# JamesYang007/adelie

Measured on AMD Instinct MI355X. Metric: lambda-paths/sec (100-lambda grpnet); HBM GB/s vs peak, higher is better.
Workload: dtype f64

## Files before the change

### adelie_amd/csrc/common.hpp

```cpp
#pragma once
#include <cstdlib>
#include <algorithm>
#include <hip/hip_runtime.h>

#include <chrono>
#include <cstdint>
#include <cstring>
#include <mutex>
#include <stdexcept>
#include <string>
#include <vector>

#include "../../include/adelie_hip.h"
#include "kernels.hpp"
#include "dev_array_host.hpp"

namespace ahip {

struct Hooks {
    long long cd_block_min_nv = -1;
    int panel_bsz = 0;
    int sparse_panel = -1;
    int std_panel = -1;
    int lookahead = -1, speculate = -1;
    int factor_sweep = -1;
    int relu_sweep = -1;
    int filter_sweep = -1;
    int filter_depth = -1;
    double filter_depth_margin = -1;
    double irls_reuse = -1;
    bool time_panel = false;
    bool cons_host = false;
    int trace = 0;
    static Hooks from_env() {
        Hooks h;
        if (const char* e = std::getenv("ADELIE_HIP_CD_BLOCK_MIN_NV")) h.cd_block_min_nv = std::atoll(e);
        if (const char* e = std::getenv("ADELIE_HIP_PANEL_BSZ")) {
            const int v = std::atoi(e);
            h.panel_bsz = (v == 32 || v == 64 || v == 128) ? v : 0;
        }
        if (const char* e = std::getenv("ADELIE_HIP_LOOKAHEAD")) h.lookahead = std::atoi(e) != 0;
        if (const char* e = std::getenv("ADELIE_HIP_SPECULATE")) h.speculate = std::atoi(e) != 0;
        if (const char* e = std::getenv("ADELIE_HIP_IRLS_REUSE")) h.irls_reuse = std::max(0.0, std::atof(e));
        h.time_panel = std::getenv("ADELIE_HIP_TIME_PANEL") != nullptr;
        if (const char* e = std::getenv("ADELIE_HIP_CONS_HOST")) h.cons_host = std::atoi(e) != 0;
        if (const char* e = std::getenv("ADELIE_HIP_SPARSE_PANEL")) h.sparse_panel = std::atoi(e) != 0;
        if (const char* e = std::getenv("ADELIE_HIP_STD_PANEL")) h.std_panel = std::atoi(e) != 0;
        if (const char* e = std::getenv("ADELIE_HIP_TRACE")) h.trace = std::max(1, std::atoi(e));
        h.factor_sweep = factor_sweep_env();
        h.relu_sweep = relu_sweep_env();
        h.filter_sweep = filter_sweep_env();
        if (const char* e = std::getenv("ADELIE_HIP_FILTER_DEPTH")) h.filter_depth = std::atoi(e) != 0;
        if (const char* e = std::getenv("ADELIE_HIP_FILTER_DEPTH_MARGIN")) h.filter_depth_margin = std::max(0.0, std::atof(e));
        return h;
    }
    static int filter_sweep_env() {
        const char* e = std::getenv("ADELIE_HIP_FILTER_SWEEP");
        return e ? int(std::atoi(e) != 0) : -1;
    }
    static int shadow_kind_env() { return shadow_kind_parse(std::getenv("ADELIE_HIP_SHADOW_KIND")); }
    static int64_t shadow_min_bytes_env() {
        const char* e = std::getenv("ADELIE_HIP_SHADOW_MIN_BYTES");
        return e ? int64_t(std::atoll(e)) : kShadowMinBytesDefault;
    }
    static int factor_sweep_env() {
        const char* e = std::getenv("ADELIE_HIP_FACTOR_SWEEP");
        return e ? int(std::atoi(e) != 0) : -1;
    }
    static int relu_sweep_env() {
        const char* e = std::getenv("ADELIE_HIP_RELU_SWEEP");
        return e ? int(std::atoi(e) != 0) : -1;
    }
};
struct SweepHooks {
    int factor = -1, relu = -1;
    static SweepHooks from_env() { return SweepHooks{Hooks::factor_sweep_env(), Hooks::relu_sweep_env()}; }
};
constexpr bool kFactorSweepDefault = false;
inline bool factor_sweep_on(int hook) { return hook < 0 ? kFactorSweepDefault : hook != 0; }
constexpr bool kReluSweepDefault = true;
inline bool relu_sweep_on(int hook) { return hook < 0 ? kReluSweepDefault : hook != 0; }
constexpr bool kReluSparseSweepDefault = true;
inline bool relu_sparse_sweep_on(int hook) { return hook < 0 ? kReluSparseSweepDefault : hook != 0; }
constexpr bool kFilterSweepDefault = true;
inline bool filter_sweep_on(int hook) { return hook < 0 ? kFilterSweepDefault : hook != 0; }
constexpr bool kFilterDepthDefault = true;
inline bool filter_depth_on(int hook) { return hook < 0 ? kFilterDepthDefault : hook != 0; }


inline core_error make_core_error(const std::string& m) { return core_error("adelie_core: " + m); }
inline core_error make_solver_error(const std::string& m) { return core_error("adelie_core solver: " + m); }

#define AHIP_CHECK(expr)                                                                                   \
    do {                                                                                                   \
        hipError_t _e = (expr);                                                                            \
        if (_e != hipSuccess)                                                                              \
            throw ::ahip::core_error(std::string("adelie_hip: HIP error '") + hipGetErrorString(_e) +     \
                                     "' at " #expr);                                                       \
    } while (0)

struct DevAllocStats {
    static double& seconds() { static double s = 0; return s; }
    static long& calls() { static long c = 0; return c; }
};

struct HostPool {
    struct Entry { size_t bytes; unsigned flags; void* p; };
    static std::mutex& mu() { static std::mutex* m = new std::mutex; return *m; }
    static std::vector<Entry>& parked() { static auto* v = new std::vector<Entry>; return *v; }
    static void* take(size_t bytes, unsigned flags) {
// ... 462 lines not shown
```

### adelie_amd/csrc/filter_host.hpp

```cpp
#pragma once
#include <algorithm>
#include <cmath>
#include <cstdint>
#include <vector>

namespace ahip {

constexpr int kFilterRuleStrong = 0, kFilterRulePivot = 1;

inline int64_t pivot_need(int64_t old_size, int64_t n_new_active, int64_t G, double subset_ratio, int64_t subset_min,
                          double slack_ratio) {
    const int64_t subset_size =
        std::min<int64_t>(std::max<int64_t>(int64_t(double(old_size) * (1 + subset_ratio)), subset_min), G);
    return subset_size + int64_t(std::ceil(slack_ratio * double(n_new_active))) + old_size + 2;
}

struct FilterRule {
    int screen_rule = kFilterRulePivot;
    double alpha = 1, lm = 0, lm_next = 0;
    bool thr_valid = false;
    double screen_thr = 0;
    int64_t thr_count = 0;
    int64_t G = 0, screen_size = 0, n_new_active = 0;
    double subset_ratio = 0.1, slack_ratio = 1.25;
// ... 18 lines not shown
    return (tstar > 0 && std::isfinite(tstar)) ? tstar : 0;
}

template <class I, class T>
inline std::vector<int32_t> filter_unpenalized_cols(const std::vector<I>& groups, const std::vector<I>& group_sizes,
                                                    const std::vector<T>& penalty) {
    std::vector<int32_t> c;
    for (size_t g = 0; g < groups.size(); ++g)
        if (!(penalty[g] > 0))
            for (I t = 0; t < group_sizes[g]; ++t) c.push_back(int32_t(groups[g] + t));
    return c;
}

constexpr int32_t kFilterOverflow = 1, kFilterStale = 2;
struct FilterFollowUp {
    bool refill;
    bool retire;
};
inline FilterFollowUp filter_follow_up(int32_t flags) {
    return FilterFollowUp{(flags & (kFilterOverflow | kFilterStale)) != 0, (flags & kFilterStale) != 0};
}
inline int64_t filter_list_cap(int64_t p) { return std::max<int64_t>(1024, p / 4); }

}
```

### adelie_amd/csrc/kernels.hpp

```cpp
#pragma once
#include <hip/hip_runtime.h>
#include <cstdint>
#include "gram_shape.hpp"
#include "multi_shape.hpp"
#include "relu_shape.hpp"
#include "relu_sparse_shape.hpp"
#include "shadow_kind_host.hpp"
#include "pieces_host.hpp"

namespace ahip {

template <class T>
struct DenseView {
    const T* X;
    int64_t n, p, ld;
};
struct SnpView {
    const uint8_t* bits;
    int64_t n, p, ldb;
};

template <class T>
struct PiecesView {
    const void* base[kMaxPieces];
// ... 74 lines not shown
void launch_shadow_build_q15(const DenseView<double>& X, int16_t* Xq, int64_t lds, double* scale, double* err, double* nrm,
                             int32_t* bad, hipStream_t s);
int filter_norm_parts(int64_t n);
struct FilteredSweep {
    const double *w, *r;
    double* v;
    double* grad;
    const double *sub_scale, *sub_vec;
    const int32_t* screen_cols;
    int64_t n_screen_cols;
    const int32_t* pen0_cols;
    int64_t n_pen0_cols;
    const int64_t *groups, *group_sizes;
    int64_t G;
    const int32_t* slot;
    const double* penalty;
    double tstar;
    double* sq_part;
    int32_t* list;
    int64_t cap;
    int32_t* meta_i;
    double* meta_d;
    double* work;
};
int64_t filtered_sweep_work_elems(int64_t n, int64_t p, int64_t n_before, int64_t cap);
void enqueue_filtered_sweep(const DenseView<double>& X, const ShadowView& S, const FilteredSweep& a, hipStream_t s);
int64_t sweep_work_elems_csc(int nb, int64_t ncols);
template <class T>
void launch_sweep_csc(const CscView<T>& X, const T* v, T* out, int64_t c0, int64_t ncols, const int32_t* cols,
                      const T* sub_scale, const T* sub_vec, bool square, T* work, hipStream_t s);
constexpr int kVecSumScratch = 8 + 256;
template <class T> void launch_vec_sum(const T* v, int64_t n, T* out, hipStream_t s);
template <class T>
void launch_std_sweep_epilogue(const T* center, const T* inv_scale, const T* raw, const T* raw_plain, const T* vsum, bool square,
                               T* out, int64_t c0, int64_t ncols, const int32_t* cols, const T* sub_scale, const T* sub_vec,
                               hipStream_t s);
template <class T>
void launch_std_gram_fix(const T* center, const T* inv_scale, T* C, int64_t ldc, int32_t M, int32_t pos0, int32_t N,
                         const int32_t* vcol, const T* m, const T* wsum, const T* xm, bool centered, hipStream_t s);
template <class T>
void launch_std_scale_coef(const T* center, const T* inv_scale, const int32_t* cols, const T* coef, const int32_t* count_dev,
                           int32_t count, T* coef2, T* kappa, hipStream_t s);
template <class T> void launch_vec_shift(T* out, int64_t n, const T* kappa, T sign, const int32_t* count_dev, hipStream_t s);
template <class T>
void launch_std_fix_gblk(T* gblk, const int32_t* cols, int nb, const T* center, const T* inv_scale, const T* rsum_dev,
                         const T* xm_view_or_null, hipStream_t s);
// ... 574 lines not shown
```

### adelie_amd/csrc/kernels_filter.hip

```cpp
#include "sweep_common.hpp"
#include <algorithm>
#include <cfloat>

namespace ahip {

namespace {

__global__ __launch_bounds__(kThreads) void shadow_build_kernel(const double* __restrict__ X, int64_t ld, int64_t n,
                                                                float* __restrict__ Xs, int64_t lds, double* __restrict__ err,
                                                                double* __restrict__ nrm, int32_t* __restrict__ bad) {
    const int64_t j = blockIdx.x;
    const int tid = threadIdx.x;
    const double* col = X + j * ld;
    float* dst = Xs + j * lds;
    double e2 = 0, n2 = 0;
    bool any_bad = false;
    for (int64_t i = tid; i < lds; i += kThreads) {
        float f = 0.f;
        if (i < n) {
            const double x = col[i];
            const bool ok = fabs(x) <= double(FLT_MAX);
            any_bad = any_bad || !ok;
            f = ok ? float(x) : 0.f;
            const double d = x - double(f);
// ... 55 lines not shown
            const double t = fmin(fmax(rint(__dmul_rn(x, inv)), -32767.0), 32767.0);
            q = int(t);
            const double d = (x - __dmul_rn(sc, t)) / sc;
            e2 = fma(d, d, e2);
            q2 = fma(t, t, q2);
        }
        dst[i] = int16_t(q);
    }
    e2 = wave_sum(e2);
    q2 = wave_sum(q2);
    if (lane == 0) { red[0][wv] = e2; red[1][wv] = q2; }
    __syncthreads();
    if (tid == 0) {
        double a = 0, b = 0;
        for (int w = 0; w < kThreads / 64; ++w) { a += red[0][w]; b += red[1][w]; }
        scale[j] = sc;
        err[j] = (sc > 0 ? sc * sqrt(a) : sqrt(double(n)) * m) * (1.0 + 1e-9);
        nrm[j] = sc * sqrt(b) * (1.0 + 1e-9);
    }
    if (any_bad) atomicOr(bad, 1);
}

__global__ __launch_bounds__(kThreads) void vmul_sq_kernel(const double* __restrict__ a, const double* __restrict__ b,
                                                           double* __restrict__ out, int64_t n, double* __restrict__ part) {
    double acc = 0;
    for (int64_t i = int64_t(blockIdx.x) * blockDim.x + threadIdx.x; i < n; i += int64_t(gridDim.x) * blockDim.x) {
        const double x = a[i] * b[i];
        out[i] = x;
        acc = fma(x, x, acc);
    }
    __shared__ double red[kThreads / 64];
    const int lane = threadIdx.x & 63, wv = threadIdx.x >> 6;
    acc = wave_sum(acc);
    if (lane == 0) red[wv] = acc;
    __syncthreads();
    if (threadIdx.x == 0) {
        double s = 0;
        for (int w = 0; w < kThreads / 64; ++w) s += red[w];
        part[blockIdx.x] = s;
    }
}

__device__ __forceinline__ void shadow_guard(double exact, double approx, int64_t j, const double* __restrict__ err,
                                             const double* __restrict__ nrm, double fp_term, const double* __restrict__ vnorm,
                                             int32_t* __restrict__ flags) {
    const double bound = (err[j] + fp_term * nrm[j]) * vnorm[0];
    if (!(fabs(exact - approx) <= bound)) atomicOr(flags, 2);
}

template <int VEC>
__device__ __forceinline__ double list_column_sum(const DenseAcc<double>& X, const double* __restrict__ v, int64_t j, int64_t r0,
                                                  int64_t r1, double* red) {
    const int tid = threadIdx.x;
    const double* cp = X.colptr(j);
    double acc = 0;
    const int64_t body_end = r0 + ((r1 - r0) / VEC) * VEC;
#pragma unroll 8
    for (int64_t i = r0 + int64_t(tid) * VEC; i < body_end; i += int64_t(kThreads) * VEC) {
        const Pack<double, VEC> vv = load_vec<double, VEC>(v + i);
        const Pack<double, VEC> xx = X.template load<VEC>(cp, i, j);
#pragma unroll
        for (int e = 0; e < VEC; ++e) acc = fma(xx.v[e], vv.v[e], acc);
    }
    for (int64_t i = body_end + tid; i < r1; i += kThreads) acc = fma(X.template load<1>(cp, i, j).v[0], v[i], acc);
    const int lane = tid & 63, wv = tid >> 6;
    const double ws = wave_sum(acc);
    if (lane == 0) red[wv] = ws;
    __syncthreads();
    double s = 0;
    if (tid == 0) {
#pragma unroll
        for (int w = 0; w < kThreads / 64; ++w) s += red[w];
    }
    return s;
}

struct ShadowF32 {
    using elem = float;
    using vec = f4_t;
    static constexpr int CB = kShadowCB, VEC = kShadowVec, kUnroll = 2;
    static constexpr bool kScaled = false, kPipelined = false;
    static constexpr int kMinWaves = 1;
    static __device__ __forceinline__ double row(vec x, int e) { return double(x[e]); }
};
typedef int i4_t __attribute__((ext_vector_type(4)));
struct ShadowQ15 {
    using elem = int16_t;
    using vec = i4_t;
    static constexpr int CB = kShadowCB16, VEC = kShadowVec16;
    static constexpr bool kScaled = true, kPipelined = true;
    static constexpr int kMinWaves = 5;
    static_assert(VEC == 8, "one 16-byte load holds 8 rows");
    static __device__ __forceinline__ double row(vec x, int e) {
        return e % 2 ? double(x[e / 2] >> 16) : double(int(int16_t(x[e / 2])));
    }
};

// ... 162 lines not shown
            out[j] = s;
        } else {
            part[int64_t(split) * max_cols + c] = s;
        }
    }
}
__global__ void sweep_list_reduce_kernel(const double* __restrict__ part, double* __restrict__ out,
                                         const int32_t* __restrict__ cols, int64_t max_cols,
                                         const int32_t* __restrict__ count_dev, int nsplit, const double* __restrict__ sub_scale,
                                         const double* __restrict__ sub_vec, const double* __restrict__ err,
                                         const double* __restrict__ nrm, double fp_term, const double* __restrict__ vnorm,
                                         int32_t* __restrict__ flags) {
    const int64_t c = int64_t(blockIdx.x) * blockDim.x + threadIdx.x;
    const int64_t count = count_dev ? min(int64_t(count_dev[0]), max_cols) : max_cols;
    if (c >= count) return;
    const int64_t j = cols[c];
    double s = 0;
    for (int r = 0; r < nsplit; ++r) s += part[int64_t(r) * max_cols + c];
    s = centred(s, j, sub_scale, sub_vec);
    if (err) shadow_guard(s, out[j], j, err, nrm, fp_term, vnorm, flags);
    out[j] = s;
}

constexpr int kClassifyThreads = 1024, kClassifyRun = 6;
__global__ __launch_bounds__(kClassifyThreads) void filter_classify_kernel(
    double* __restrict__ grad, const int64_t* __restrict__ groups, const int64_t* __restrict__ group_sizes, int64_t G,
    const int32_t* __restrict__ slot, const double* __restrict__ penalty, double tstar, const double* __restrict__ err,
    const double* __restrict__ nrm, double fp_term, const double* __restrict__ sq_part, int n_part,
    const double* __restrict__ sub_scale, const double* __restrict__ sub_vec, const double* __restrict__ stage,
    const int32_t* __restrict__ xa, int64_t na, const int32_t* __restrict__ xb, int64_t nb, int x_nsplit,
    int32_t* __restrict__ list, int64_t cap, int32_t* __restrict__ meta_i, double* __restrict__ meta_d) {
    constexpr int NW = kClassifyThreads / 64, R = kClassifyRun;
    __shared__ double sred[NW];
    __shared__ int32_t wtot[NW];
    __shared__ double s_vnorm;
    __shared__ int32_t s_first[kClassifyThreads * R], s_want[kClassifyThreads * R];
    const int tid = threadIdx.x, lane = tid & 63, wv = tid >> 6;
    {
        double a = 0;
        for (int i = tid; i < n_part; i += kClassifyThreads) a += sq_part[i];
        a = wave_sum(a);
        if (lane == 0) sred[wv] = a;
        __syncthreads();
        if (tid == 0) {
            double s = 0;
            for (int w = 0; w < NW; ++w) s += sred[w];
            s_vnorm = sqrt(s) * (1.0 + 1e-6);
            meta_d[0] = s_vnorm;
            meta_d[1] = sub_scale ? sub_scale[0] : 0.0;
            meta_i[1] = 0;
            meta_i[3] = 0;
        }
        __syncthreads();
    }
    const double vnorm = s_vnorm;
    const int64_t ne = na + nb;
    for (int pass = 0; pass < 2; ++pass) {
        const int32_t* xl = pass ? xb : xa;
        const int64_t c0 = pass ? na : 0, cnt = pass ? nb : na;
        for (int64_t c = tid; c < cnt; c += kClassifyThreads) {
            const int64_t j = xl[c];
            double s = 0;
            for (int r = 0; r < x_nsplit; ++r) s += stage[int64_t(r) * ne + c0 + c];
            s = centred(s, j, sub_scale, sub_vec);
            shadow_guard(s, grad[j], j, err, nrm, fp_term, &s_vnorm, meta_i + 1);
            grad[j] = s;
        }
        __syncthreads();
    }
    int64_t run = 0;
    for (int64_t base = 0; base < G; base += int64_t(kClassifyThreads) * R) {
        int32_t k[R], sz[R];
        double thr[R], a2[R], b2[R];
        {
            int32_t sl[R];
            double pn[R];
            int64_t kk[R], ss[R];
#pragma unroll
// ... 9 lines not shown
            for (int u = 0; u < R; ++u) {
                const bool on = base + int64_t(u) * kClassifyThreads + tid < G && sl[u] < 0 && pn[u] > 0 && ss[u] > 0;
                k[u] = int32_t(kk[u]);
                sz[u] = on ? int32_t(ss[u]) : 0;
                thr[u] = tstar * pn[u];
                a2[u] = 0;
                b2[u] = 0;
            }
        }
        int32_t longest = 0;
#pragma unroll
        for (int u = 0; u < R; ++u) longest = max(longest, sz[u]);
        for (int32_t t = 0; t < longest; ++t) {
            double x[R], e[R], m[R];
#pragma unroll
            for (int u = 0; u < R; ++u) {
                const int64_t at = t < sz[u] ? int64_t(k[u]) + t : 0;
                x[u] = grad[at];
                e[u] = err[at];
                m[u] = nrm[at];
            }
#pragma unroll
            for (int u = 0; u < R; ++u)
                if (t < sz[u]) {
                    const double b = e[u] + fp_term * m[u];
                    a2[u] = fma(x[u], x[u], a2[u]);
                    b2[u] = fma(b, b, b2[u]);
                }
        }
#pragma unroll
        for (int u = 0; u < R; ++u) {
            if (sz[u] > 0) {
                const double reach = (sqrt(a2[u]) + sqrt(b2[u]) * vnorm * (1.0 + 1e-9)) * (1.0 + 1e-9);
                if (reach < thr[u]) sz[u] = 0;
            }
            s_first[u * kClassifyThreads + tid] = k[u];
            s_want[u * kClassifyThreads + tid] = sz[u];
        }
        __syncthreads();
        int32_t mine = 0;
#pragma unroll
        for (int u = 0; u < R; ++u) mine += s_want[tid * R + u];
        int32_t inc = mine;
#pragma unroll
        for (int off = 1; off < 64; off <<= 1) {
            const int32_t y = __shfl_up(inc, off, 64);
            if (lane >= off) inc += y;
        }
        if (lane == 63) wtot[wv] = inc;
        __syncthreads();
        int32_t before = 0, total = 0;
        for (int w = 0; w < NW; ++w) {
            const int32_t t = wtot[w];
            if (w < wv) before += t;
            total += t;
        }
        int64_t at = run + before + inc - mine;
        if (mine > 0)
// ... 45 lines not shown
                       const int32_t* count_dev, const double* sub_scale, const double* sub_vec, const ShadowView& guard,
                       const double* vnorm, int32_t* flags, double* work, hipStream_t s) {
    if (max_cols <= 0) return;
    DenseAcc<double> acc{X.X, X.ld};
    const ListShape L = list_shape(X, v);
    const auto kernel = L.vec ? sweep_list_kernel<VecOf<double>::N> : sweep_list_kernel<1>;
    hipLaunchKernelGGL(kernel, dim3((unsigned)max_cols, (unsigned)L.ns), dim3(kThreads), 0, s, acc, v, out, work, X.n, cols,
                       max_cols, count_dev, L.rps, L.ns, sub_scale, sub_vec, guard.err, guard.nrm, guard.fp_term(), vnorm, flags);
    if (L.ns > 1)
        hipLaunchKernelGGL(sweep_list_reduce_kernel, dim3((unsigned)((max_cols + 255) / 256)), dim3(256), 0, s, work, out, cols,
                           max_cols, count_dev, L.ns, sub_scale, sub_vec, guard.err, guard.nrm, guard.fp_term(), vnorm, flags);
}
int64_t shadow_work_elems(int64_t n, int64_t p) {
    int64_t blocks_c, rps;
    int ns, ns16;
    sweep_shape(n, p, kShadowVec, blocks_c, ns, rps, kShadowCB);
    sweep_shape(n, p, kShadowVec16, blocks_c, ns16, rps, kShadowCB16);
    return int64_t(std::max(ns, ns16)) * p + 16;
}
int64_t list_work_elems(int64_t n, int64_t p, int64_t max_cols) {
    int64_t blocks_c, rps;
    int ns;
    sweep_shape(n, p, 1, blocks_c, ns, rps);
    return int64_t(ns) * max_cols + 16;
}
template <class Kind, int XVEC>
void launch_shadow_sweep(const DenseView<double>& X, const ShadowView& S, const FilteredSweep& a, int64_t na, int64_t nb,
                         const ListShape& L, double* stage, hipStream_t s) {
    int64_t blocks_c, rps;
    int ns;
    sweep_shape(S.n, S.p, Kind::VEC, blocks_c, ns, rps, Kind::CB);
    hipLaunchKernelGGL((shadow_sweep_kernel<Kind, XVEC>), dim3((unsigned)((na + nb) * L.ns + blocks_c * ns)), dim3(kThreads), 0, s,
                       static_cast<const typename Kind::elem*>(S.X), S.ld, S.scale, a.v, ns == 1 ? a.grad : a.work, S.n, S.p,
                       blocks_c, rps, ns, a.sub_scale, a.sub_vec, DenseAcc<double>{X.X, X.ld}, a.screen_cols, na, a.pen0_cols, nb,
                       L.rps, L.ns, stage);
    if (ns > 1) launch_sweep_reduce<double>(a.work, a.grad, S.p, ns, 0, nullptr, a.sub_scale, a.sub_vec, s);
}
}

int64_t filtered_sweep_work_elems(int64_t n, int64_t p, int64_t n_before, int64_t cap) {
    return shadow_work_elems(n, p) + list_work_elems(n, p, std::max(n_before, cap));
}
void enqueue_filtered_sweep(const DenseView<double>& X, const ShadowView& S, const FilteredSweep& a, hipStream_t s) {
    if (S.p <= 0) return;
    const int64_t na = a.screen_cols ? a.n_screen_cols : 0, nb = a.pen0_cols ? a.n_pen0_cols : 0;
    double* stage = a.work + shadow_work_elems(S.n, S.p);
    hipLaunchKernelGGL(vmul_sq_kernel, dim3(grid1d(S.n, kThreads, 1024)), dim3(kThreads), 0, s, a.w, a.r, a.v, S.n, a.sq_part);
    const ListShape L = list_shape(X, a.v);
    constexpr int V = VecOf<double>::N;
    if (S.kind == kShadowQ15) {
        if (L.vec) launch_shadow_sweep<ShadowQ15, V>(X, S, a, na, nb, L, stage, s);
        else launch_shadow_sweep<ShadowQ15, 1>(X, S, a, na, nb, L, stage, s);
    } else {
        if (L.vec) launch_shadow_sweep<ShadowF32, V>(X, S, a, na, nb, L, stage, s);
        else launch_shadow_sweep<ShadowF32, 1>(X, S, a, na, nb, L, stage, s);
    }
    hipLaunchKernelGGL(filter_classify_kernel, dim3(1), dim3(kClassifyThreads), 0, s, a.grad, a.groups, a.group_sizes, a.G, a.slot,
                       a.penalty, a.tstar, S.err, S.nrm, S.fp_term(), a.sq_part, filter_norm_parts(S.n), a.sub_scale, a.sub_vec,
                       stage, a.screen_cols, na, a.pen0_cols, nb, L.ns, a.list, a.cap, a.meta_i, a.meta_d);
    launch_sweep_list(X, a.v, a.grad, a.list, a.cap, a.meta_i, a.sub_scale, a.sub_vec, S, a.meta_d, a.meta_i + 1, stage, s);
}

}
```

### adelie_amd/csrc/solver.hip

```cpp
#include "common.hpp"
#include "design_ops.hpp"
#include "filter_host.hpp"
#include "screen_reads_host.hpp"
#include "cox.hpp"

#include <algorithm>
#include <cstring>
#include <exception>
#include <type_traits>
#include <chrono>
#include <condition_variable>
#include <mutex>
#include <thread>
#include <cmath>
#include <cstdio>
#include <cstdlib>
#include <limits>
#include <numeric>
#include <unordered_set>

namespace ahip {
void set_last_error(const std::string& s);
double g_hessian_min = 1e-24;
double g_dbeta_tol = 1e-12;
// ... 801 lines not shown
        const int n_part = filter_norm_parts(n);
        dpart.reserve(n_part);
        work.reserve(size_t(std::max(filtered_sweep_work_elems(n, p, int64_t(scols.size() + pen0.size()), cap), sweep_work_elems(n, p))));
        dw.upload(w, n, s); dr.upload(r, n, s); dsc.upload(&sub_scale, 1, s); dpen.upload(penalty, G, s);
        dgroups.upload(groups, G, s); dgs.upload(group_sizes, G, s); dslot.upload(slot.data(), G, s);
        if (sub_vec) { dxm.reserve(p); dxm.upload(sub_vec, p, s); }
        if (!scols.empty()) { dscols.reserve(scols.size()); dscols.upload(scols.data(), scols.size(), s); }
        if (!pen0.empty()) { dpen0.reserve(pen0.size()); dpen0.upload(pen0.data(), pen0.size(), s); }
        const double* xm = sub_vec ? dxm.p : nullptr;
        const DenseView<double> X = d->dense<double>();
        int32_t meta[4] = {0, 0, 0, 0};
        std::vector<int32_t> list;
        if (!route) {
            launch_vmul<double>(dw.p, dr.p, dv.p, n, s);
            launch_sweep<double>(X, dv.p, dgrad.p, 0, p, nullptr, dsc.p, xm, false, work.p, s);
            std::fill(exact, exact + p, uint8_t(1));
        } else {
            FilteredSweep a{};
            a.w = dw.p; a.r = dr.p; a.v = dv.p; a.grad = dgrad.p; a.sub_scale = dsc.p; a.sub_vec = xm;
            a.screen_cols = scols.empty() ? nullptr : dscols.p; a.n_screen_cols = int64_t(scols.size());
            a.pen0_cols = pen0.empty() ? nullptr : dpen0.p; a.n_pen0_cols = int64_t(pen0.size());
            a.groups = dgroups.p; a.group_sizes = dgs.p; a.G = G; a.slot = dslot.p; a.penalty = dpen.p; a.tstar = tstar;
            a.sq_part = dpart.p; a.list = dlist.p; a.cap = cap; a.meta_i = dmeta.p; a.meta_d = dmetad.p; a.work = work.p;
            enqueue_filtered_sweep(X, sh, a, s);
            AHIP_CHECK(hipMemcpyAsync(meta, dmeta.p, sizeof(meta), hipMemcpyDeviceToHost, s));
            AHIP_CHECK(hipStreamSynchronize(s));
            list.resize(size_t(meta[0]));
            if (meta[0] > 0) AHIP_CHECK(hipMemcpyAsync(list.data(), dlist.p, size_t(meta[0]) * sizeof(int32_t), hipMemcpyDeviceToHost, s));
            std::fill(exact, exact + p, uint8_t(0));
        }
        AHIP_CHECK(hipMemcpyAsync(grad, dgrad.p, size_t(p) * sizeof(double), hipMemcpyDeviceToHost, s));
        AHIP_CHECK(hipStreamSynchronize(s));
        if (route) {
            for (int32_t c : scols) exact[c] = 1;
            for (int32_t c : pen0) exact[c] = 1;
            for (int32_t c : list) exact[c] = 1;
            if (meta[1] & 2) adelie_hip_internal_shadow_mark_stale(d);
        }
        info[0] = meta[0]; info[1] = meta[1]; info[2] = route ? 1 : 0; info[3] = meta[2];
    } catch (const std::exception& e) {
        set_last_error(e.what());
        return 1;
    }
    return 0;
}

// ... 682 lines not shown
```

### adelie_amd/csrc/solver_screen.hpp

```cpp
    void sweep(const T* v, T* out, const int32_t* cols, idx ncols, const T* sub_scale, const T* sub_vec,
               bool square = false) {
        if (multi()) {
            if (cols || ncols != p || sub_vec || square) throw make_core_error("unsupported sweep on a multi-response view.");
            const MultiView<T> mv = D->multi<T>();
            launch_multi_sweep<T>(mv, v, out, d_work_sweep.reserve(size_t(multi_sweep_work_elems<T>(mv))), st);
            return;
        }
        if (std_generic()) {
            const T* ce = static_cast<const T*>(D->std_center);
            const T* is = static_cast<const T*>(D->std_iscale);
            T* tmp = d_std_tmp.reserve(size_t(2 * ncols + kVecSumScratch));
            T *raw = tmp, *raw_plain = tmp + ncols, *vsum = tmp + 2 * ncols;
            T* work = d_work_sweep.reserve(size_t(raw_sweep_work_elems(*D, ncols, false)));
            raw_sweep<T>(*D, v, raw, 0, ncols, cols, nullptr, nullptr, square, false, work, st);
            if (square) raw_sweep<T>(*D, v, raw_plain, 0, ncols, cols, nullptr, nullptr, false, false, work, st);
            launch_vec_sum<T>(v, n, vsum, st);
            launch_std_sweep_epilogue<T>(ce, is, raw, raw_plain, vsum, square, out, 0, ncols, cols, sub_scale, sub_vec, st);
            return;
        }
        if (batcher && dense() && !cols && ncols == p && !square &&
            batcher->template sweep<T>(D->dense<T>(), v, out, sub_scale, sub_vec, st)) {
            ++cnt.n_sweeps_shared;
            return;
        }
// ... 366 lines not shown
        if constexpr (std::is_same<T, double>::value) {
            const T* xm = intercept ? d_xm.p : nullptr;
            const int64_t cap = fs_cap();
            if (fs_pen0_cols < 0) {
                const std::vector<int32_t> c0 = filter_unpenalized_cols(groups, group_sizes, penalty);
                fs_pen0_cols = int64_t(c0.size());
                if (!c0.empty()) {
                    d_fs_pen0.reserve(c0.size());
                    d_fs_pen0.upload(c0.data(), c0.size(), st);
                }
            }
            d_fs_part.reserve(size_t(filter_norm_parts(n)));
            d_fs_meta.reserve(4);
            d_fs_metad.reserve(2);
            d_fs_list.reserve(size_t(cap));
            d_fs_work.reserve(size_t(filtered_sweep_work_elems(n, p, int64_t(nv) + fs_pen0_cols, cap)));
            FilteredSweep a{};
            a.w = d_w.p; a.r = d_r.p; a.v = d_v.p; a.grad = d_grad.p; a.sub_scale = rsum_dev; a.sub_vec = xm;
            a.screen_cols = nv > 0 ? d_vcol.p : nullptr; a.n_screen_cols = nv;
            a.pen0_cols = fs_pen0_cols > 0 ? d_fs_pen0.p : nullptr; a.n_pen0_cols = fs_pen0_cols;
            a.groups = d_groups.p; a.group_sizes = d_gsizes.p; a.G = G; a.slot = d_slot.p; a.penalty = d_penalty.p; a.tstar = tstar;
            a.sq_part = d_fs_part.p; a.list = d_fs_list.p; a.cap = cap; a.meta_i = d_fs_meta.p; a.meta_d = d_fs_metad.p;
            a.work = d_fs_work.p;
            t_fsweep.begin(st);
            enqueue_filtered_sweep(D->dense<T>(), fs_shadow, a, st);
            t_fsweep.end(st);
            d_fs_meta.download(fs_meta, 4, st);
            grad_filtered = true;
            fs_lm = lm;
            fs_pending_screen_cols = int64_t(nv) + std::max<int64_t>(fs_pen0_cols, 0);
            ++n_sweeps_filtered;
        }
    }

    void filtered_sweep_arrived() {
        if (!grad_filtered) return;
        const int64_t exact = fs_pending_screen_cols + fs_meta[0];
        n_filter_exact_cols += exact;
        n_filter_open_cols += fs_meta[0];
        if (hooks.trace)
            std::fprintf(stderr, "[fsweep] lmda %.6g screen+pen0 cols %lld open %d wanted %d flags %d predicted open %lld\n",
                         double(fs_lm), (long long)fs_pending_screen_cols, int(fs_meta[0]), int(fs_meta[2]), int(fs_meta[1]),
                         (long long)depth_open_cols);
        n_filter_shadow_cols += int64_t(p);
        fsweep_bytes += double(n) * (double(exact) * 8.0 + double(p) * fs_shadow.elem_bytes());
        const FilterFollowUp fu = filter_follow_up(fs_meta[1]);
// ... 595 lines not shown
```

Before: 5.057.

## Parallelize filtered-sweep classify across chunk blocks and wave-split list sweep

Replaces the single-block filter classify kernel with a multi-block chunked classifier that writes per-chunk candidate lists, uses a last-block ticket to finalize metadata, and feeds a new list sweep kernel that splits each column across 64-thread waves with unrolled loads. It also sizes the list-sweep grid from the predicted open-column depth instead of the full cap. The goal is to remove the serial single-block bottleneck and the over-launched list sweep in the filtered gradient step. In exchange it adds atomics and cross-block coordination, a larger work buffer, and more complex indexing via the chunk prefix lookup.

```diff
diff --git a/adelie_amd/csrc/common.hpp b/adelie_amd/csrc/common.hpp
--- a/adelie_amd/csrc/common.hpp
+++ b/adelie_amd/csrc/common.hpp
@@ -27,6 +27,7 @@
     int relu_sweep = -1;
     int filter_sweep = -1;
     int filter_depth = -1;
+    int filter_tail = -1;
     double filter_depth_margin = -1;
     double irls_reuse = -1;
     bool time_panel = false;
@@ -50,6 +51,7 @@
         h.factor_sweep = factor_sweep_env();
         h.relu_sweep = relu_sweep_env();
         h.filter_sweep = filter_sweep_env();
+        h.filter_tail = filter_tail_env();
         if (const char* e = std::getenv("ADELIE_HIP_FILTER_DEPTH")) h.filter_depth = std::atoi(e) != 0;
         if (const char* e = std::getenv("ADELIE_HIP_FILTER_DEPTH_MARGIN")) h.filter_depth_margin = std::max(0.0, std::atof(e));
         return h;
@@ -57,6 +59,14 @@
     static int filter_sweep_env() {
         const char* e = std::getenv("ADELIE_HIP_FILTER_SWEEP");
         return e ? int(std::atoi(e) != 0) : -1;
+    }
+    static int filter_tail_env() {
+        const char* e = std::getenv("ADELIE_HIP_FILTER_TAIL");
+        return e ? int(std::atoi(e) != 0) : -1;
+    }
+    static int64_t filter_list_grid_env() {
+        const char* e = std::getenv("ADELIE_HIP_FILTER_LIST_GRID");
+        return e ? std::max<int64_t>(0, int64_t(std::atoll(e))) : 0;
     }
     static int shadow_kind_env() { return shadow_kind_parse(std::getenv("ADELIE_HIP_SHADOW_KIND")); }
     static int64_t shadow_min_bytes_env() {
@@ -86,6 +96,8 @@
 inline bool filter_sweep_on(int hook) { return hook < 0 ? kFilterSweepDefault : hook != 0; }
 constexpr bool kFilterDepthDefault = true;
 inline bool filter_depth_on(int hook) { return hook < 0 ? kFilterDepthDefault : hook != 0; }
+constexpr bool kFilterTailDefault = true;
+inline bool filter_tail_on(int hook) { return hook < 0 ? kFilterTailDefault : hook != 0; }
 
 
 inline core_error make_core_error(const std::string& m) { return core_error("adelie_core: " + m); }
diff --git a/adelie_amd/csrc/filter_host.hpp b/adelie_amd/csrc/filter_host.hpp
--- a/adelie_amd/csrc/filter_host.hpp
+++ b/adelie_amd/csrc/filter_host.hpp
@@ -64,4 +64,38 @@
 }
 inline int64_t filter_list_cap(int64_t p) { return std::max<int64_t>(1024, p / 4); }
 
+constexpr int kTailThreads = 256, kTailMaxChunks = 64;
+struct TailChunks {
+    int64_t chunk_groups;
+    int nchunk;
+};
+inline TailChunks tail_chunks(int64_t G) {
+    G = std::max<int64_t>(G, 1);
+    const int64_t per = (G + kTailMaxChunks - 1) / kTailMaxChunks;
+    const int64_t cg = (per + kTailThreads - 1) / kTailThreads * kTailThreads;
+    return TailChunks{cg, int((G + cg - 1) / cg)};
 }
+inline void tail_prefix(const int32_t* counts, int nchunk, int64_t cap, int32_t* incl) {
+    int64_t run = 0;
+    for (int k = 0; k < nchunk; ++k) {
+        run += counts[k];
+        incl[k] = int32_t(std::min(run, cap));
+    }
+}
+#if defined(__HIPCC__)
+#define AHIP_FILTER_HD __host__ __device__
+#else
+#define AHIP_FILTER_HD
+#endif
+struct TailEntry {
+    int chunk;
+    int32_t offset;
+};
+AHIP_FILTER_HD inline TailEntry tail_locate(const int32_t* incl, int nchunk, int32_t c) {
+    int k = 0;
+    for (int i = 0; i < nchunk; ++i) k += incl[i] <= c ? 1 : 0;
+    return TailEntry{k, c - (k > 0 ? incl[k - 1] : 0)};
+}
+constexpr int kListUnroll = 24;
+
+}
diff --git a/adelie_amd/csrc/kernels.hpp b/adelie_amd/csrc/kernels.hpp
--- a/adelie_amd/csrc/kernels.hpp
+++ b/adelie_amd/csrc/kernels.hpp
@@ -120,6 +120,8 @@
     int32_t* meta_i;
     double* meta_d;
     double* work;
+    bool chunked_tail = true;
+    int64_t list_grid = 0;
 };
 int64_t filtered_sweep_work_elems(int64_t n, int64_t p, int64_t n_before, int64_t cap);
 void enqueue_filtered_sweep(const DenseView<double>& X, const ShadowView& S, const FilteredSweep& a, hipStream_t s);
diff --git a/adelie_amd/csrc/kernels_filter.hip b/adelie_amd/csrc/kernels_filter.hip
--- a/adelie_amd/csrc/kernels_filter.hip
+++ b/adelie_amd/csrc/kernels_filter.hip
@@ -1,4 +1,5 @@
 #include "sweep_common.hpp"
+#include "filter_host.hpp"
 #include <algorithm>
 #include <cfloat>
 
@@ -101,7 +102,12 @@
 }
 
 __global__ __launch_bounds__(kThreads) void vmul_sq_kernel(const double* __restrict__ a, const double* __restrict__ b,
-                                                           double* __restrict__ out, int64_t n, double* __restrict__ part) {
+                                                           double* __restrict__ out, int64_t n, double* __restrict__ part,
+                                                           int32_t* __restrict__ zero, int32_t* __restrict__ ticket) {
+    if (zero && blockIdx.x == 0 && threadIdx.x == 0) {
+        zero[0] = 0;
+        ticket[0] = 0;
+    }
     double acc = 0;
     for (int64_t i = int64_t(blockIdx.x) * blockDim.x + threadIdx.x; i < n; i += int64_t(gridDim.x) * blockDim.x) {
         const double x = a[i] * b[i];
@@ -120,11 +126,31 @@
     }
 }
 
+__device__ __forceinline__ void shadow_guard_loaded(double exact, double approx, double ej, double mj, double fp_term, double vn,
+                                                    int32_t* __restrict__ flags) {
+    const double bound = (ej + fp_term * mj) * vn;
+    if (!(fabs(exact - approx) <= bound)) atomicOr(flags, 2);
+}
 __device__ __forceinline__ void shadow_guard(double exact, double approx, int64_t j, const double* __restrict__ err,
                                              const double* __restrict__ nrm, double fp_term, const double* __restrict__ vnorm,
                                              int32_t* __restrict__ flags) {
-    const double bound = (err[j] + fp_term * nrm[j]) * vnorm[0];
-    if (!(fabs(exact - approx) <= bound)) atomicOr(flags, 2);
+    shadow_guard_loaded(exact, approx, err[j], nrm[j], fp_term, vnorm[0], flags);
+}
+
+__device__ __forceinline__ double list_column_finish(const DenseAcc<double>& X, const double* __restrict__ v, const double* cp,
+                                                     int64_t j, int64_t body_end, int64_t r1, double acc, double* red) {
+    const int tid = threadIdx.x;
+    for (int64_t i = body_end + tid; i < r1; i += kThreads) acc = fma(X.template load<1>(cp, i, j).v[0], v[i], acc);
+    const int lane = tid & 63, wv = tid >> 6;
+    const double ws = wave_sum(acc);
+    if (lane == 0) red[wv] = ws;
+    __syncthreads();
+    double s = 0;
+    if (tid == 0) {
+#pragma unroll
+        for (int w = 0; w < kThreads / 64; ++w) s += red[w];
+    }
+    return s;
 }
 
 template <int VEC>
@@ -141,17 +167,53 @@
 #pragma unroll
         for (int e = 0; e < VEC; ++e) acc = fma(xx.v[e], vv.v[e], acc);
     }
-    for (int64_t i = body_end + tid; i < r1; i += kThreads) acc = fma(X.template load<1>(cp, i, j).v[0], v[i], acc);
-    const int lane = tid & 63, wv = tid >> 6;
-    const double ws = wave_sum(acc);
-    if (lane == 0) red[wv] = ws;
-    __syncthreads();
-    double s = 0;
-    if (tid == 0) {
-#pragma unroll
-        for (int w = 0; w < kThreads / 64; ++w) s += red[w];
-    }
-    return s;
+    return list_column_finish(X, v, cp, j, body_end, r1, acc, red);
+}
+
+template <int VEC>
+__device__ __forceinline__ double list_wave_sum(const DenseAcc<double>& X, const double* __restrict__ v, int64_t j, int64_t r0,
+                                                int64_t r1, int wave) {
+    constexpr int U = kListUnroll;
+    constexpr int64_t kStep = int64_t(kThreads) * VEC;
+    const int tid = wave * 64 + int(threadIdx.x);
+    const double* cp = X.colptr(j);
+    double acc = 0;
+    const int64_t body_end = r0 + ((r1 - r0) / VEC) * VEC;
+    int64_t i = r0 + int64_t(tid) * VEC;
+    for (; i + (U - 1) * kStep < body_end; i += U * kStep) {
+        Pack<double, VEC> xx[U], vv[U];
+#pragma unroll
+        for (int k = 0; k < U; ++k) {
+            xx[k] = X.template load<VEC>(cp, i + k * kStep, j);
+            vv[k] = load_vec<double, VEC>(v + i + k * kStep);
+        }
+        __builtin_amdgcn_sched_barrier(0);
+#pragma unroll
+        for (int k = 0; k < U; ++k) {
+#pragma unroll
+            for (int e = 0; e < VEC; ++e) acc = fma(xx[k].v[e], vv[k].v[e], acc);
+        }
+        __builtin_amdgcn_sched_barrier(0);
+    }
+    if (i < body_end) {
+        Pack<double, VEC> xx[U], vv[U];
+#pragma unroll
+        for (int k = 0; k < U; ++k) {
+            const int64_t at = i + k * kStep < body_end ? i + k * kStep : i;
+            xx[k] = X.template load<VEC>(cp, at, j);
+            vv[k] = load_vec<double, VEC>(v + at);
+        }
+        __builtin_amdgcn_sched_barrier(0);
+#pragma unroll
+        for (int k = 0; k < U; ++k) {
+            if (i + k * kStep < body_end) {
+#pragma unroll
+                for (int e = 0; e < VEC; ++e) acc = fma(xx[k].v[e], vv[k].v[e], acc);
+            }
+        }
+    }
+    for (int64_t t = body_end + tid; t < r1; t += kThreads) acc = fma(X.template load<1>(cp, t, j).v[0], v[t], acc);
+    return wave_sum(acc);
 }
 
 struct ShadowF32 {
@@ -360,6 +422,213 @@
     out[j] = s;
 }
 
+constexpr int kVnormWaves = 16;
+template <int NT>
+__device__ __forceinline__ double inflated_vnorm(const double* __restrict__ sq_part, int n_part, double* sred, double* out) {
+    const int tid = threadIdx.x, lane = tid & 63;
+    for (int w = tid >> 6; w < kVnormWaves; w += NT / 64) {
+        double a = 0;
+        for (int i = w * 64 + lane; i < n_part; i += kVnormWaves * 64) a += sq_part[i];
+        a = wave_sum(a);
+        if (lane == 0) sred[w] = a;
+    }
+    __syncthreads();
+    if (tid == 0) {
+        double s = 0;
+        for (int w = 0; w < kVnormWaves; ++w) s += sred[w];
+        out[0] = sqrt(s) * (1.0 + 1e-6);
+    }
+    __syncthreads();
+    return out[0];
+}
+__device__ __forceinline__ void reach_add(double& a2, double& b2, double x, double e, double m, double fp_term) {
+    const double b = e + fp_term * m;
+    a2 = fma(x, x, a2);
+    b2 = fma(b, b, b2);
+}
+__device__ __forceinline__ bool reach_below(double a2, double b2, double vnorm, double thr) {
+    const double reach = (sqrt(a2) + sqrt(b2) * vnorm * (1.0 + 1e-9)) * (1.0 + 1e-9);
+    return reach < thr;
+}
+
+constexpr int kTailCounts = 2, kTailFirst = kTailCounts + kTailMaxChunks, kTailHeader = kTailFirst + kTailMaxChunks;
+int64_t tail_work_elems(int64_t p) { return (kTailHeader + p + 1) / 2 + 1; }
+constexpr int64_t kListGridMin = 256;
+
+__device__ __forceinline__ void chunk_prefix(const int32_t* __restrict__ tail, int nchunk, int64_t cap, int32_t* s_incl) {
+    const int tid = threadIdx.x;
+    if (tid < 64) {
+        int64_t inc = tid < nchunk ? int64_t(tail[kTailCounts + tid]) : 0;
+#pragma unroll
+        for (int off = 1; off < 64; off <<= 1) {
+            const int64_t y = __shfl_up(inc, off, 64);
+            if (tid >= off) inc += y;
+        }
+        s_incl[tid] = int32_t(inc < cap ? inc : cap);
+    }
+    __syncthreads();
+}
+
+struct StagedColumn {
+    double s0, g, e, m, cv;
+};
+__device__ __forceinline__ StagedColumn staged_load(const double* __restrict__ part0, const double* grad, const double* __restrict__ err,
+                                                    const double* __restrict__ nrm, const double* __restrict__ sub_vec, int64_t j) {
+    return StagedColumn{part0[0], grad[j], err[j], nrm[j], sub_vec ? sub_vec[j] : 0.0};
+}
+
+__global__ __launch_bounds__(kTailThreads) void chunk_filter_classify_kernel(
+    double* __restrict__ grad, const int64_t* __restrict__ groups, const int64_t* __restrict__ group_sizes, int64_t G,
+    int64_t chunk_groups, const int32_t* __restrict__ slot, const double* __restrict__ penalty, double tstar,
+    const double* __restrict__ err, const double* __restrict__ nrm, double fp_term, const double* __restrict__ sq_part, int n_part,
+    const double* __restrict__ sub_scale, const double* __restrict__ sub_vec, const double* __restrict__ stage,
+    const int32_t* __restrict__ xa, int64_t na, const int32_t* __restrict__ xb, int64_t nb, int x_nsplit, int32_t* __restrict__ tail,
+    int64_t p, int64_t cap, int32_t* __restrict__ meta_i, double* __restrict__ meta_d) {
+    constexpr int NW = kTailThreads / 64;
+    __shared__ double sred[kVnormWaves];
+    __shared__ double s_vnorm;
+    __shared__ int32_t wtot[NW];
+    __shared__ int32_t s_last;
+    const int tid = threadIdx.x, lane = tid & 63, wv = tid >> 6;
+    const int64_t g0 = int64_t(blockIdx.x) * chunk_groups, g1 = min(G, g0 + chunk_groups);
+    const int64_t g_me = min(g0 + tid, g1 - 1);
+    int32_t sl = slot[g_me];
+    double pn = penalty[g_me];
+    int64_t k = groups[g_me], ss = group_sizes[g_me];
+    const int64_t col0 = groups[g0], col1 = groups[g1 - 1] + group_sizes[g1 - 1];
+    const int64_t c_me = int64_t(blockIdx.x) * kTailThreads + tid;
+    const int64_t ne = na + nb, c_step = int64_t(gridDim.x) * kTailThreads;
+    int32_t j_a = 0, j_b = 0;
+    if (c_me < na) j_a = xa[c_me];
+    if (c_me < nb) j_b = xb[c_me];
+    const double vnorm = inflated_vnorm<kTailThreads>(sq_part, n_part, sred, &s_vnorm);
+    int32_t sz = g0 + tid < g1 && sl < 0 && pn > 0 && ss > 0 ? int32_t(ss) : 0;
+    double x0 = 0, e0 = 0, m0 = 0;
+    if (sz > 0) x0 = grad[k], e0 = err[k], m0 = nrm[k];
+    StagedColumn first_a{}, first_b{};
+    if (c_me < na) first_a = staged_load(stage + c_me, grad, err, nrm, sub_vec, j_a);
+    if (c_me < nb) first_b = staged_load(stage + na + c_me, grad, err, nrm, sub_vec, j_b);
+    for (int pass = 0; pass < 2; ++pass) {
+        const int32_t* xl = pass ? xb : xa;
+        const int64_t c0 = pass ? na : 0, cnt = pass ? nb : na;
+        for (int64_t c = c_me; c < cnt; c += c_step) {
+            const int64_t j = c == c_me ? (pass ? j_b : j_a) : xl[c];
+            const StagedColumn o = c == c_me ? (pass ? first_b : first_a) : staged_load(stage + c0 + c, grad, err, nrm, sub_vec, j);
+            double sum = 0.0 + o.s0;
+            for (int r = 1; r < x_nsplit; ++r) sum += stage[int64_t(r) * ne + c0 + c];
+            if (sub_vec) sum -= sub_scale[0] * o.cv;
+            shadow_guard_loaded(sum, o.g, o.e, o.m, fp_term, vnorm, meta_i + 1);
+            grad[j] = sum;
+        }
+        __syncthreads();
+    }
+    const int64_t seg = col0 >= 0 ? min(col1, p) - col0 : 0;
+    int32_t* mylist = tail + kTailHeader + col0;
+    int64_t run = 0;
+    for (int64_t base = g0; base < g1; base += kTailThreads) {
+        if (base != g0) {
+            const bool in = base + tid < g1;
+            const int64_t g = in ? base + tid : g1 - 1;
+            sl = slot[g], pn = penalty[g], k = groups[g], ss = group_sizes[g];
+            sz = in && sl < 0 && pn > 0 && ss > 0 ? int32_t(ss) : 0;
+            if (sz > 0) x0 = grad[k], e0 = err[k], m0 = nrm[k];
+        }
+        double a2 = 0, b2 = 0;
+        if (sz > 0) reach_add(a2, b2, x0, e0, m0, fp_term);
+        for (int32_t t = 1; t < sz; ++t) reach_add(a2, b2, grad[k + t], err[k + t], nrm[k + t], fp_term);
+        if (sz > 0 && reach_below(a2, b2, vnorm, tstar * pn)) sz = 0;
+        int32_t inc = sz;
+#pragma unroll
+        for (int off = 1; off < 64; off <<= 1) {
+            const int32_t y = __shfl_up(inc, off, 64);
+            if (lane >= off) inc += y;
+        }
+        if (lane == 63) wtot[wv] = inc;
+        __syncthreads();
+        int32_t before = 0, total = 0;
+#pragma unroll
+        for (int w = 0; w < NW; ++w) {
+            const int32_t t = wtot[w];
+            if (w < wv) before += t;
+            total += t;
+        }
+        const int64_t at = run + before + inc - sz;
+        for (int32_t t = 0; t < sz; ++t)
+            if (at + t < seg) mylist[at + t] = int32_t(k) + t;
+        run += total;
+        __syncthreads();
+    }
+    run = min(run, max(seg, int64_t(0)));
+    if (tid == 0) {
+        __hip_atomic_store(tail + kTailCounts + blockIdx.x, int32_t(run < int64_t(0x7fffffff) ? run : int64_t(0x7fffffff)),
+                           __ATOMIC_RELAXED, __HIP_MEMORY_SCOPE_AGENT);
+        __hip_atomic_store(tail + kTailFirst + blockIdx.x, int32_t(col0), __ATOMIC_RELAXED, __HIP_MEMORY_SCOPE_AGENT);
+        const int32_t ticket = __hip_atomic_fetch_add(tail, 1, __ATOMIC_ACQ_REL, __HIP_MEMORY_SCOPE_AGENT);
+        s_last = ticket == int32_t(gridDim.x) - 1;
+    }
+    __syncthreads();
+    if (s_last && wv == 0) {
+        int64_t total = lane < int(gridDim.x) ? int64_t(__hip_atomic_load(tail + kTailCounts + lane, __ATOMIC_RELAXED, __HIP_MEMORY_SCOPE_AGENT)) : 0;
+#pragma unroll
+        for (int off = 32; off > 0; off >>= 1) total += __shfl_down(total, off, 64);
+        if (lane == 0) {
+            meta_i[0] = int32_t(total < cap ? total : cap);
+            if (total > cap) atomicOr(meta_i + 1, 1);
+            meta_i[2] = int32_t(total < int64_t(0x7fffffff) ? total : int64_t(0x7fffffff));
+            meta_i[3] = 0;
+            meta_d[0] = vnorm;
+            meta_d[1] = sub_scale ? sub_scale[0] : 0.0;
+        }
+    }
+}
+
+constexpr int kListWaves = kThreads / 64;
+template <int VEC>
+__global__ __launch_bounds__(64) void chunk_sweep_list_kernel(DenseAcc<double> X, const double* __restrict__ v,
+                                                              double* __restrict__ part, int64_t n,
+                                                              const int32_t* __restrict__ tail, int nchunk, int64_t max_cols,
+                                                              int64_t rows_per_split) {
+    __shared__ int32_t s_incl[kTailMaxChunks];
+    chunk_prefix(tail, nchunk, max_cols, s_incl);
+    const int lane = threadIdx.x, wave = blockIdx.x % kListWaves;
+    const int32_t total = s_incl[kTailMaxChunks - 1];
+    const int split = blockIdx.y;
+    const int64_t r0 = int64_t(split) * rows_per_split;
+    for (int32_t c = blockIdx.x / kListWaves; c < total; c += gridDim.x / kListWaves) {
+        const int k = __popcll(__ballot(s_incl[lane] <= c));
+        const int32_t off = c - (k > 0 ? s_incl[k - 1] : 0);
+        const int64_t j = __builtin_amdgcn_readfirstlane(tail[kTailHeader + tail[kTailFirst + k] + off]);
+        const double s = list_wave_sum<VEC>(X, v, j, r0, min(n, r0 + rows_per_split), wave);
+        if (lane == 0) part[(int64_t(split) * kListWaves + wave) * max_cols + c] = s;
+    }
+}
+__global__ __launch_bounds__(256) void chunk_sweep_list_reduce_kernel(const double* __restrict__ part, double* __restrict__ out,
+                                                                      const int32_t* __restrict__ tail, int nchunk, int64_t max_cols,
+                                                                      int32_t* __restrict__ cols_out, int nsplit,
+                                                                      const double* __restrict__ sub_scale,
+                                                                      const double* __restrict__ sub_vec, const double* __restrict__ err,
+                                                                      const double* __restrict__ nrm, double fp_term,
+                                                                      const double* __restrict__ vnorm, int32_t* __restrict__ flags) {
+    __shared__ int32_t s_incl[kTailMaxChunks];
+    chunk_prefix(tail, nchunk, max_cols, s_incl);
+    const int32_t total = s_incl[kTailMaxChunks - 1];
+    for (int64_t c = int64_t(blockIdx.x) * blockDim.x + threadIdx.x; c < total; c += int64_t(gridDim.x) * blockDim.x) {
+        const TailEntry at = tail_locate(s_incl, nchunk, int32_t(c));
+        const int64_t j = tail[kTailHeader + tail[kTailFirst + at.chunk] + at.offset];
+        double s = 0;
+        for (int r = 0; r < nsplit; ++r) {
+            double sr = 0;
+#pragma unroll
+            for (int w = 0; w < kListWaves; ++w) sr += part[(int64_t(r) * kListWaves + w) * max_cols + c];
+            s = nsplit == 1 ? sr : s + sr;
+        }
+        s = centred(s, j, sub_scale, sub_vec);
+        shadow_guard(s, out[j], j, err, nrm, fp_term, vnorm, flags);
+        out[j] = s;
+        cols_out[c] = int32_t(j);
+    }
+}
+
 constexpr int kClassifyThreads = 1024, kClassifyRun = 6;
 __global__ __launch_bounds__(kClassifyThreads) void filter_classify_kernel(
     double* __restrict__ grad, const int64_t* __restrict__ groups, const int64_t* __restrict__ group_sizes, int64_t G,
@@ -374,24 +643,14 @@
     __shared__ double s_vnorm;
     __shared__ int32_t s_first[kClassifyThreads * R], s_want[kClassifyThreads * R];
     const int tid = threadIdx.x, lane = tid & 63, wv = tid >> 6;
-    {
-        double a = 0;
-        for (int i = tid; i < n_part; i += kClassifyThreads) a += sq_part[i];
-        a = wave_sum(a);
-        if (lane == 0) sred[wv] = a;
-        __syncthreads();
-        if (tid == 0) {
-            double s = 0;
-            for (int w = 0; w < NW; ++w) s += sred[w];
-            s_vnorm = sqrt(s) * (1.0 + 1e-6);
-            meta_d[0] = s_vnorm;
-            meta_d[1] = sub_scale ? sub_scale[0] : 0.0;
-            meta_i[1] = 0;
-            meta_i[3] = 0;
-        }
-        __syncthreads();
-    }
-    const double vnorm = s_vnorm;
+    const double vnorm = inflated_vnorm<kClassifyThreads>(sq_part, n_part, sred, &s_vnorm);
+    if (tid == 0) {
+        meta_d[0] = vnorm;
+        meta_d[1] = sub_scale ? sub_scale[0] : 0.0;
+        meta_i[1] = 0;
+        meta_i[3] = 0;
+    }
+    __syncthreads();
     const int64_t ne = na + nb;
     for (int pass = 0; pass < 2; ++pass) {
         const int32_t* xl = pass ? xb : xa;
@@ -447,18 +706,11 @@
             }
 #pragma unroll
             for (int u = 0; u < R; ++u)
-                if (t < sz[u]) {
-                    const double b = e[u] + fp_term * m[u];
-                    a2[u] = fma(x[u], x[u], a2[u]);
-                    b2[u] = fma(b, b, b2[u]);
-                }
+                if (t < sz[u]) reach_add(a2[u], b2[u], x[u], e[u], m[u], fp_term);
         }
 #pragma unroll
         for (int u = 0; u < R; ++u) {
-            if (sz[u] > 0) {
-                const double reach = (sqrt(a2[u]) + sqrt(b2[u]) * vnorm * (1.0 + 1e-9)) * (1.0 + 1e-9);
-                if (reach < thr[u]) sz[u] = 0;
-            }
+            if (sz[u] > 0 && reach_below(a2[u], b2[u], vnorm, thr[u])) sz[u] = 0;
             s_first[u * kClassifyThreads + tid] = k[u];
             s_want[u * kClassifyThreads + tid] = sz[u];
         }
@@ -550,7 +802,7 @@
     int64_t blocks_c, rps;
     int ns;
     sweep_shape(n, p, 1, blocks_c, ns, rps);
-    return int64_t(ns) * max_cols + 16;
+    return int64_t(ns) * kListWaves * max_cols + 16;
 }
 template <class Kind, int XVEC>
 void launch_shadow_sweep(const DenseView<double>& X, const ShadowView& S, const FilteredSweep& a, int64_t na, int64_t nb,
@@ -564,16 +816,30 @@
                        L.rps, L.ns, stage);
     if (ns > 1) launch_sweep_reduce<double>(a.work, a.grad, S.p, ns, 0, nullptr, a.sub_scale, a.sub_vec, s);
 }
+void launch_chunk_sweep_list(const DenseView<double>& X, const double* v, double* out, const int32_t* tail, int nchunk,
+                             int64_t max_cols, int64_t grid, int32_t* cols_out, const double* sub_scale, const double* sub_vec,
+                             const ShadowView& guard, const double* vnorm, int32_t* flags, double* work, hipStream_t s) {
+    if (max_cols <= 0) return;
+    DenseAcc<double> acc{X.X, X.ld};
+    const ListShape L = list_shape(X, v);
+    const auto kernel = L.vec ? chunk_sweep_list_kernel<VecOf<double>::N> : chunk_sweep_list_kernel<1>;
+    hipLaunchKernelGGL(kernel, dim3((unsigned)(grid * kListWaves), (unsigned)L.ns), dim3(64), 0, s, acc, v, work, X.n, tail, nchunk,
+                       max_cols, L.rps);
+    hipLaunchKernelGGL(chunk_sweep_list_reduce_kernel, dim3((unsigned)((grid + 255) / 256)), dim3(256), 0, s, work, out, tail, nchunk,
+                       max_cols, cols_out, L.ns, sub_scale, sub_vec, guard.err, guard.nrm, guard.fp_term(), vnorm, flags);
+}
 }
 
 int64_t filtered_sweep_work_elems(int64_t n, int64_t p, int64_t n_before, int64_t cap) {
-    return shadow_work_elems(n, p) + list_work_elems(n, p, std::max(n_before, cap));
+    return shadow_work_elems(n, p) + list_work_elems(n, p, std::max(n_before, cap)) + tail_work_elems(p);
 }
 void enqueue_filtered_sweep(const DenseView<double>& X, const ShadowView& S, const FilteredSweep& a, hipStream_t s) {
     if (S.p <= 0) return;
     const int64_t na = a.screen_cols ? a.n_screen_cols : 0, nb = a.pen0_cols ? a.n_pen0_cols : 0;
     double* stage = a.work + shadow_work_elems(S.n, S.p);
-    hipLaunchKernelGGL(vmul_sq_kernel, dim3(grid1d(S.n, kThreads, 1024)), dim3(kThreads), 0, s, a.w, a.r, a.v, S.n, a.sq_part);
+    int32_t* tail = reinterpret_cast<int32_t*>(stage + list_work_elems(S.n, S.p, std::max(na + nb, a.cap)));
+    hipLaunchKernelGGL(vmul_sq_kernel, dim3(grid1d(S.n, kThreads, 1024)), dim3(kThreads), 0, s, a.w, a.r, a.v, S.n, a.sq_part,
+                       a.chunked_tail ? a.meta_i + 1 : nullptr, tail);
     const ListShape L = list_shape(X, a.v);
     constexpr int V = VecOf<double>::N;
     if (S.kind == kShadowQ15) {
@@ -583,6 +849,17 @@
         if (L.vec) launch_shadow_sweep<ShadowF32, V>(X, S, a, na, nb, L, stage, s);
         else launch_shadow_sweep<ShadowF32, 1>(X, S, a, na, nb, L, stage, s);
     }
+    if (a.chunked_tail) {
+        const TailChunks C = tail_chunks(a.G);
+        hipLaunchKernelGGL(chunk_filter_classify_kernel, dim3((unsigned)C.nchunk), dim3(kTailThreads), 0, s, a.grad, a.groups,
+                           a.group_sizes, a.G, C.chunk_groups, a.slot, a.penalty, a.tstar, S.err, S.nrm, S.fp_term(), a.sq_part,
+                           filter_norm_parts(S.n), a.sub_scale, a.sub_vec, stage, a.screen_cols, na, a.pen0_cols, nb, L.ns, tail,
+                           S.p, a.cap, a.meta_i, a.meta_d);
+        const int64_t grid = a.list_grid > 0 ? std::min(a.cap, std::max(a.list_grid, kListGridMin)) : a.cap;
+        launch_chunk_sweep_list(X, a.v, a.grad, tail, C.nchunk, a.cap, grid, a.list, a.sub_scale, a.sub_vec, S, a.meta_d,
+                                a.meta_i + 1, stage, s);
+        return;
+    }
     hipLaunchKernelGGL(filter_classify_kernel, dim3(1), dim3(kClassifyThreads), 0, s, a.grad, a.groups, a.group_sizes, a.G, a.slot,
                        a.penalty, a.tstar, S.err, S.nrm, S.fp_term(), a.sq_part, filter_norm_parts(S.n), a.sub_scale, a.sub_vec,
                        stage, a.screen_cols, na, a.pen0_cols, nb, L.ns, a.list, a.cap, a.meta_i, a.meta_d);
diff --git a/adelie_amd/csrc/solver.hip b/adelie_amd/csrc/solver.hip
--- a/adelie_amd/csrc/solver.hip
+++ b/adelie_amd/csrc/solver.hip
@@ -847,6 +847,8 @@
             a.pen0_cols = pen0.empty() ? nullptr : dpen0.p; a.n_pen0_cols = int64_t(pen0.size());
             a.groups = dgroups.p; a.group_sizes = dgs.p; a.G = G; a.slot = dslot.p; a.penalty = dpen.p; a.tstar = tstar;
             a.sq_part = dpart.p; a.list = dlist.p; a.cap = cap; a.meta_i = dmeta.p; a.meta_d = dmetad.p; a.work = work.p;
+            a.chunked_tail = filter_tail_on(Hooks::filter_tail_env());
+            a.list_grid = Hooks::filter_list_grid_env();
             enqueue_filtered_sweep(X, sh, a, s);
             AHIP_CHECK(hipMemcpyAsync(meta, dmeta.p, sizeof(meta), hipMemcpyDeviceToHost, s));
             AHIP_CHECK(hipStreamSynchronize(s));
diff --git a/adelie_amd/csrc/solver_screen.hpp b/adelie_amd/csrc/solver_screen.hpp
--- a/adelie_amd/csrc/solver_screen.hpp
+++ b/adelie_amd/csrc/solver_screen.hpp
@@ -412,6 +412,8 @@
             a.groups = d_groups.p; a.group_sizes = d_gsizes.p; a.G = G; a.slot = d_slot.p; a.penalty = d_penalty.p; a.tstar = tstar;
             a.sq_part = d_fs_part.p; a.list = d_fs_list.p; a.cap = cap; a.meta_i = d_fs_meta.p; a.meta_d = d_fs_metad.p;
             a.work = d_fs_work.p;
+            a.chunked_tail = filter_tail_on(hooks.filter_tail);
+            a.list_grid = depth_rule() ? depth_open_cols + depth_open_cols / 8 : 0;
             t_fsweep.begin(st);
             enqueue_filtered_sweep(D->dense<T>(), fs_shadow, a, st);
             t_fsweep.end(st);
```

New measurement: 5.097 (median of 6 runs). No clear change (+0.8%).
